# ZooMEISTER/vickers-hardness-Unet

Measured on AMD Instinct MI355X. Metric: 512x512 images/sec (train fwd+bwd), higher is better.
Workload: dtype bf16

## Files before the change

### vickers-hardness-unet_amd/csrc/conv_halo.hip

```cpp
#include <stdlib.h>
#include <string.h>

#include <string>
#include <type_traits>

#include "vk_common.h"

#ifdef VK_STAMP
#define VK_T(var) { __builtin_amdgcn_sched_barrier(0); const unsigned long long t_ = __builtin_amdgcn_s_memtime(); __builtin_amdgcn_s_waitcnt(0xC07F); __builtin_amdgcn_sched_barrier(0); var = t_; }
#else
#define VK_T(var)
#endif

namespace vk {

struct HaloSrc {
  const void* ptr;
  const float* scale;
  const float* shift;
  int C, up, relu;
  uint32_t bytes;
};

#ifndef VK_EPI_BATCH_READS
// ... 1294 lines not shown
  const uint32_t slab_bytes = (uint32_t)p.K * 64u;
  const uint32_t lane16 = (uint32_t)lane * 16u;
  auto dma_b = [&](int cc, int s, int buf) {
#pragma unroll
    for (int i = 0; i < Cfg::DMAW; ++i) {
      const int pc = wave + i * NW;
      const int r = pc / (BN / 16), sub = pc - r * (BN / 16);
      const int tap = p.flip ? 8 - (3 * r + s) : 3 * r + s;
      const uint32_t goff = (uint32_t)(cc * 9 + tap) * slab_bytes + (uint32_t)(n0 + sub * 16) * 64u;
      char* dst = Bbuf + buf * Cfg::B_BYTES + (r * BN + sub * 16) * 64;
      __builtin_amdgcn_raw_ptr_buffer_load_lds(rsw, (lds_void*)dst, 16, lane16, goff, 0, 0);
    }
  };

  const int wrow0 = (wave / WGN) * TP;
  const int wch0 = (wave % WGN) * (TC * 16);
  f32x4_t acc[TC][TP];
#pragma unroll
  for (int a = 0; a < TC; ++a)
#pragma unroll
    for (int b = 0; b < TP; ++b) acc[a][b] = f32x4_t{0.f, 0.f, 0.f, 0.f};
  const int li = lane & 15, kg = lane >> 4;
  const int a_lane = (wrow0 * 18 + li) * APS + kg * 16;
  const int b_lane = (wch0 + li) * 64 + ((kg ^ swz(li)) << 4);

  u32x4_t X[TP + 2], W0[TC], W1[TC], W2[TC];
  auto rd = [](const char* q) { return *reinterpret_cast<const u32x4_t*>(q); };
  auto mfma_row = [&](const u32x4_t (&Wr)[TC], int r) {
#pragma unroll
    for (int a = 0; a < TC; ++a)
#pragma unroll
      for (int b = 0; b < TP; ++b) acc[a][b] = Mma<T>::run(Wr[a], X[b + r], acc[a][b]);
  };
  constexpr int NM = TC * TP * (sizeof(T) == 4 ? 4 : 1);
  constexpr int kWaitAll = 0x0070;
  constexpr int kWaitLds = 0xC07F;

#ifdef VK_STAMP
  unsigned long long t_begin, t_pro, tkX = 0, tkW = 0, tkB1 = 0, tkY = 0, tkB2 = 0;
  VK_T(t_begin)
#endif
  const int ksp = p.ksplit > 1 ? p.ksplit : 1;
  const int c_begin = (int)((long)p.nchunks * blockIdx.z / ksp), c_end = (int)((long)p.nchunks * (blockIdx.z + 1) / ksp);
  load_halo(c_begin);
  dma_b(c_begin, 0, 0);
  dma_b(c_begin, 1, 1);
  dma_b(c_begin, 2, 2);
  store_halo(Abuf);
  __syncthreads();
#pragma unroll
  for (int h = 0; h < TP; ++h) X[h] = rd(Abuf + a_lane + h * (18 * APS));
#pragma unroll
  for (int a = 0; a < TC; ++a) W0[a] = rd(Bbuf + b_lane + (a * 16) * 64);

  VK_T(t_pro)
  const bool late = wave >= NW / 2;
  if (late) {
    asm volatile("" ::: "memory");
    __builtin_amdgcn_s_waitcnt(kWaitLds);
    __builtin_amdgcn_s_barrier();
    asm volatile("" ::: "memory");
  }
  for (int cc = c_begin; cc < c_end; ++cc) {
    const bool next_chunk = cc + 1 < c_end;
    const char* const Acur = Abuf + ((cc - c_begin) & 1) * Cfg::A_BYTES + a_lane;
    char* const Anext = Abuf + ((cc - c_begin + 1) & 1) * Cfg::A_BYTES;
#pragma unroll
    for (int s = 0; s < 3; ++s) {
      const int st = 3 * (cc - c_begin) + s;
      const char* const As = Acur + s * APS;
      const char* const Bs = Bbuf + (st & 3) * Cfg::B_BYTES + b_lane;
      const bool more = s < 2 || next_chunk;
      const char* const An = s < 2 ? Acur + (s + 1) * APS : Anext + a_lane;
      const char* const Bn = Bbuf + ((st + 1) & 3) * Cfg::B_BYTES + b_lane;
#ifdef VK_STAMP
      unsigned long long t0, t1, t2, t3, t4, t5;
#endif
      VK_T(t0)
      X[TP] = rd(As + TP * (18 * APS));
#pragma unroll
      for (int a = 0; a < TC; ++a) W1[a] = rd(Bs + (BN + a * 16) * 64);
      X[TP + 1] = rd(As + (TP + 1) * (18 * APS));
#pragma unroll
      for (int a = 0; a < TC; ++a) W2[a] = rd(Bs + (2 * BN + a * 16) * 64);
      mfma_row(W0, 0);
      mfma_row(W1, 1);
      mfma_row(W2, 2);
      __builtin_amdgcn_sched_group_barrier(0x100, 2 + 2 * TC, 0);
      __builtin_amdgcn_sched_group_barrier(0x008, 3 * NM, 0);
      VK_T(t1)
      asm volatile("" ::: "memory");
      __builtin_amdgcn_s_waitcnt(kWaitAll);
      VK_T(t2)
      __builtin_amdgcn_s_barrier();
      asm volatile("" ::: "memory");
      VK_T(t3)
      if (p.dbg & 16) __builtin_amdgcn_s_setprio(1);
      if (more) {
#pragma unroll
        for (int h = 0; h < TP; ++h) X[h] = rd(An + h * (18 * APS));
#pragma unroll
        for (int a = 0; a < TC; ++a) W0[a] = rd(Bn + (a * 16) * 64);
      }
      __builtin_amdgcn_sched_barrier(0);
      if (next_chunk) {
        if (s == 0) load_halo(cc + 1);
        if (s == 1) store_halo(Anext);
        dma_b(cc + 1, s, (st + 3) & 3);
      }
      asm volatile("" ::: "memory");
      __builtin_amdgcn_s_waitcnt(kWaitLds);
      if (p.dbg & 16) __builtin_amdgcn_s_setprio(0);
      VK_T(t4)
      __builtin_amdgcn_s_barrier();
      asm volatile("" ::: "memory");
      VK_T(t5)
#ifdef VK_STAMP
      tkX += t1 - t0; tkW += t2 - t1; tkB1 += t3 - t2; tkY += t4 - t3; tkB2 += t5 - t4;
#endif
    }
  }
  if (!late) {
    asm volatile("" ::: "memory");
    __builtin_amdgcn_s_barrier();
    asm volatile("" ::: "memory");
  }
  __builtin_amdgcn_s_waitcnt(kWaitAll);
#ifdef VK_STAMP
  {
    unsigned long long t_end;
    VK_T(t_end)
    if (p.stamps && lane == 0) {
      unsigned long long* o = p.stamps + ((size_t)(blockIdx.y * gridDim.x + blockIdx.x) * NW + wave) * 8;
      o[0] = tkX; o[1] = tkW; o[2] = tkB1; o[3] = tkY; o[4] = tkB2; o[5] = t_pro - t_begin; o[6] = t_end - t_begin; o[7] = 3 * (c_end - c_begin);
    }
  }
#endif
  __syncthreads();

  if (p.ksplit > 1) {
    float* sl = p.slab + (size_t)blockIdx.z * ((size_t)p.N * p.H * p.W * p.K);
#pragma unroll
    for (int a = 0; a < TC; ++a)
#pragma unroll
      for (int b = 0; b < TP; ++b) {
        const int y = y0 + wrow0 + b, x = x0 + li, ch = n0 + wch0 + a * 16 + kg * 4;
        if (y < p.H && x < p.W && ch < p.K) *reinterpret_cast<f32x4_t*>(sl + (((size_t)n * p.H + y) * p.W + x) * p.K + ch) = acc[a][b];
      }
    return;
  }
  halo_epilogue<T, TH, BN, TP, TC, NT, (BN <= 64 && TH == 16)>(smem, acc, p, n, y0, x0, n0, wrow0, wch0);
}

template <typename T, int TH, int BN, int WGM, int WGN, int MINW>
__global__ __launch_bounds__(64 * WGM * WGN, MINW) void conv3x3_colp_kernel(const HaloParams p) {
  using Cfg = ColCfg<T, TH, BN, WGM, WGN, false>;
  constexpr int EB = Cfg::EB, VE = Cfg::VE, CK = Cfg::CK, HPIX = Cfg::HPIX, NPV = Cfg::NPV, NT = Cfg::NT, NW = Cfg::NW;
  constexpr int TP = Cfg::TP, TC = Cfg::TC, APS = Cfg::APS, NPIECE = Cfg::NPIECE;
  typedef __attribute__((address_space(3))) void lds_void;

  extern __shared__ __attribute__((aligned(16))) char smem[];
  char* const Abuf = smem;
  char* const Bbuf = smem + Cfg::A_BYTES;
  const int tid = threadIdx.x, lane = tid & 63;
  const int wave = __builtin_amdgcn_readfirstlane(tid >> 6);
  const int nsp = p.N * p.tiles_y * p.tiles_x;
  const int total = nsp * p.kyn;
  const bool xcd_runs = (nsp & 7) == 0 && (gridDim.x & 7) == 0 && p.kyn == 1;

  const __amdgpu_buffer_rsrc_t rs0 = make_rsrc(p.s0.ptr, p.s0.bytes);
  const __amdgpu_buffer_rsrc_t rs1 = make_rsrc(p.s1.ptr ? p.s1.ptr : p.s0.ptr, p.s1.ptr ? p.s1.bytes : 0u);
  const __amdgpu_buffer_rsrc_t rsw = make_rsrc(p.w, p.w_bytes);

  const int hv = tid & 3;
  const int hgrp = halo_group(tid);
  const int Hh = p.H >> 1, Wh = p.W >> 1;
  struct TileGeo { int n, y0, x0, n0; };
  auto decode = [&](int t) {
    TileGeo g;
    const int ky = t % p.kyn;
    int bt = t / p.kyn;
    if (xcd_runs) bt = (bt & 7) * (nsp >> 3) + (bt >> 3);
    const int tx = bt % p.tiles_x;
    bt /= p.tiles_x;
    const int ty = bt % p.tiles_y;
    g.n = bt / p.tiles_y;
    g.y0 = ty * TH; g.x0 = tx * 16; g.n0 = ky * BN;
    return g;
  };
  auto halo_index = [&](const TileGeo& g, int (&hf)[NPV], int (&hh)[NPV]) {
#pragma unroll
    for (int i = 0; i < NPV; ++i) {
      const int hp = hgrp + i * (NT / 4);
      const int hy = hp / 18, hx = hp - hy * 18;
      const int y = g.y0 - 1 + hy, x = g.x0 - 1 + hx;
      const bool ok = hp < HPIX && (unsigned)y < (unsigned)p.H && (unsigned)x < (unsigned)p.W;
      hf[i] = ok ? (g.n * p.H + y) * p.W + x : -1;
      hh[i] = ok ? (g.n * Hh + (y >> 1)) * Wh + (x >> 1) : -1;
    }
  };
  int h_full[NPV], h_half[NPV], h_full_n[NPV], h_half_n[NPV];
  u32x4_t areg[NPV];
  float sc[VE], sh[VE];
  bool aff = false, relu = false;

  auto load_halo = [&](int cc, const int (&hf)[NPV], const int (&hh)[NPV]) {
    const int c = cc * CK;
    const bool first = c < p.s0.C;
    const HaloSrc& sd = first ? p.s0 : p.s1;
    const int cl = (first ? c : c - p.s0.C) + hv * VE;
    aff = sd.scale != nullptr;
    relu = sd.relu != 0;
    if (aff) {
#pragma unroll
      for (int j = 0; j < VE; j += 4) {
        const f32x4_t s4 = *reinterpret_cast<const f32x4_t*>(sd.scale + cl + j);
        const f32x4_t h4 = *reinterpret_cast<const f32x4_t*>(sd.shift + cl + j);
#pragma unroll
        for (int e = 0; e < 4; ++e) { sc[j + e] = s4[e]; sh[j + e] = h4[e]; }
      }
    }
    const bool up = sd.up != 0;
#pragma unroll
    for (int i = 0; i < NPV; ++i) {
      const int pix = up ? hh[i] : hf[i];
      const uint32_t off = (uint32_t)(pix * sd.C + cl) * (uint32_t)EB;
      if (first) areg[i] = buf_load16(rs0, pix >= 0 ? off : kOOB);
      else areg[i] = buf_load16(rs1, pix >= 0 ? off : kOOB);
    }
  };
  auto store_halo = [&](char* A, const int (&hf)[NPV]) {
#pragma unroll
    for (int i = 0; i < NPV; ++i) {
      const int hp = hgrp + i * (NT / 4);
      if (hp >= HPIX) continue;
      u32x4_t v = areg[i];
      if (aff) {
        v = AffineRelu<T>::run(v, sc, sh, relu);
        if (hf[i] < 0) v = u32x4_t{0, 0, 0, 0};
      }
      *reinterpret_cast<u32x4_t*>(A + hp * APS + hv * 16) = v;
    }
  };
  const uint32_t slab_bytes = (uint32_t)p.K * 64u;
  const uint32_t lane16 = (uint32_t)lane * 16u;
  auto dma_b = [&](int n0, int cc, int s, int buf) {
#pragma unroll
    for (int i = 0; i < (NPIECE + NW - 1) / NW; ++i) {
      const int pc = wave + i * NW;
      if (NPIECE % NW == 0 || pc < NPIECE) {
        const int r = pc / (BN / 16), sub = pc - r * (BN / 16);
        const int tap = p.flip ? 8 - (3 * r + s) : 3 * r + s;
        const uint32_t goff = (uint32_t)(cc * 9 + tap) * slab_bytes + (uint32_t)(n0 + sub * 16) * 64u;
        char* dst = Bbuf + buf * Cfg::B_BYTES + (r * BN + sub * 16) * 64;
        __builtin_amdgcn_raw_ptr_buffer_load_lds(rsw, (lds_void*)dst, 16, lane16, goff, 0, 0);
      }
    }
  };

  const int wrow0 = (wave / WGN) * TP;
  const int wch0 = (wave % WGN) * (TC * 16);
  const int li = lane & 15, kg = lane >> 4;
  const int a_lane = (wrow0 * 18 + li) * APS + kg * 16;
  const int b_lane = (wch0 + li) * 64 + ((kg ^ swz(li)) << 4);
  f32x4_t acc[TC][TP];

  auto compute = [&](const char* A, const char* B) {
    u32x4_t X[TP + 2], W[3][TC];
#pragma unroll
    for (int h = 0; h < TP + 2; ++h) X[h] = *reinterpret_cast<const u32x4_t*>(A + h * (18 * APS));
#pragma unroll
    for (int r = 0; r < 3; ++r)
#pragma unroll
      for (int a = 0; a < TC; ++a) W[r][a] = *reinterpret_cast<const u32x4_t*>(B + (r * BN + a * 16) * 64);
#pragma unroll
    for (int r = 0; r < 3; ++r)
#pragma unroll
      for (int a = 0; a < TC; ++a)
#pragma unroll
        for (int b = 0; b < TP; ++b) acc[a][b] = Mma<T>::run(W[r][a], X[b + r], acc[a][b]);
    constexpr int NM = TC * TP * (sizeof(T) == 4 ? 4 : 1);
    __builtin_amdgcn_sched_group_barrier(0x100, TP + 2 + TC, 0);
    __builtin_amdgcn_sched_group_barrier(0x100, TC, 0);
    __builtin_amdgcn_sched_group_barrier(0x008, NM, 0);
    __builtin_amdgcn_sched_group_barrier(0x100, TC, 0);
    __builtin_amdgcn_sched_group_barrier(0x008, NM, 0);
    __builtin_amdgcn_sched_group_barrier(0x008, NM, 0);
  };

  int t = blockIdx.x;
  if (t >= total) return;
  TileGeo g = decode(t);
  halo_index(g, h_full, h_half);
  load_halo(0, h_full, h_half);
  double dsum[2] = {0.0, 0.0};
  int st = 0;
  for (;;) {
    dma_b(g.n0, 0, 0, st & 1);
    store_halo(Abuf, h_full);
    __syncthreads();
#pragma unroll
    for (int a = 0; a < TC; ++a)
#pragma unroll
      for (int b = 0; b < TP; ++b) acc[a][b] = f32x4_t{0.f, 0.f, 0.f, 0.f};
    const int tn = t + (int)gridDim.x;
    const bool more_tiles = tn < total;
    TileGeo gn = g;
    const char* const A = Abuf + a_lane;
    auto stage = [&](int cc, auto s_c, auto last_c) {
      constexpr int s = decltype(s_c)::value;
      constexpr bool LAST = decltype(last_c)::value;
      if (s < 2) dma_b(g.n0, cc, s + 1, (st + 1) & 1);
      else if (!LAST) dma_b(g.n0, cc + 1, 0, (st + 1) & 1);
      if (s == 0 && !LAST) load_halo(cc + 1, h_full, h_half);
      if (s == 2 && LAST && more_tiles) {
        gn = decode(tn);
        halo_index(gn, h_full_n, h_half_n);
        load_halo(0, h_full_n, h_half_n);
      }
      compute(A + s * APS, Bbuf + (st & 1) * Cfg::B_BYTES + b_lane);
      if (s == 2 && !LAST) {
        __syncthreads();
        store_halo(Abuf, h_full);
      }
      __syncthreads();
      ++st;
    };
    using I0 = std::integral_constant<int, 0>;
    using I1 = std::integral_constant<int, 1>;
    using I2 = std::integral_constant<int, 2>;
    for (int cc = 0; cc + 1 < p.nchunks; ++cc) {
      stage(cc, I0{}, std::false_type{});
      stage(cc, I1{}, std::false_type{});
      stage(cc, I2{}, std::false_type{});
    }
    stage(p.nchunks - 1, I0{}, std::true_type{});
    stage(p.nchunks - 1, I1{}, std::true_type{});
    stage(p.nchunks - 1, I2{}, std::true_type{});
    constexpr bool DEFER = VK_COLP_DEFER_STATS && (sizeof(T) == 2 || BN < 64);
    halo_epilogue<T, TH, BN, TP, TC, NT, (BN <= 64 && TH == 16)>(smem, acc, p, g.n, g.y0, g.x0, g.n0, wrow0, wch0, 0, 0, DEFER ? dsum : nullptr);
    if (DEFER && (!more_tiles || gn.n0 != g.n0)) stats_flush<BN>(p, g.n0, dsum);
    if (!more_tiles) break;
    __syncthreads();
    t = tn;
    g = gn;
#pragma unroll
    for (int i = 0; i < NPV; ++i) { h_full[i] = h_full_n[i]; h_half[i] = h_half_n[i]; }
  }
}

struct StemTile {
  static constexpr int ROWS = 37, VPR = 20, PITCH = VPR * 16;
  static constexpr int A_BYTES = ROWS * PITCH;
  static constexpr int W_OFF = (A_BYTES + 1023) / 1024 * 1024, W_BYTES = 28 * 1024;
};

template <typename T>
__global__ __launch_bounds__(256, 3) void stem7x7_kernel(const HaloParams p) {
  using Cfg = ColCfg<T, 16, 64, 4, 1, false>;
  static_assert(sizeof(T) == 2, "16-bit types: a pixel of the NHWC4 input is 8 bytes");
  constexpr int NV = (StemTile::ROWS * StemTile::VPR + 255) / 256;
  extern __shared__ __attribute__((aligned(16))) char smem[];
  const int tid = threadIdx.x, lane = tid & 63;
  const int wave = __builtin_amdgcn_readfirstlane(tid >> 6);
  int bt = blockIdx.x;
  if ((gridDim.x & 7) == 0) bt = (bt & 7) * (int)(gridDim.x >> 3) + (bt >> 3);
  const int tx = bt % p.tiles_x;
  bt /= p.tiles_x;
  const int ty = bt % p.tiles_y;
  const int n = bt / p.tiles_y;
  const int y0 = ty * 16, x0 = tx * 16;
  const __amdgpu_buffer_rsrc_t rs0 = make_rsrc(p.s0.ptr, p.s0.bytes);
  const __amdgpu_buffer_rsrc_t rsw = make_rsrc(p.w, p.w_bytes);

  u32x4_t areg[NV];
#pragma unroll
  for (int i = 0; i < NV; ++i) {
    const int v = tid + i * 256;
    const int ry = v / StemTile::VPR, vc = v - ry * StemTile::VPR;
    const int y = 2 * y0 - 3 + ry, x = 2 * x0 - 4 + 2 * vc;
    const bool ok = v < StemTile::ROWS * StemTile::VPR && (unsigned)y < (unsigned)p.Hi && (unsigned)x < (unsigned)p.Wi;
    areg[i] = buf_load16(rs0, ok ? (uint32_t)((n * p.Hi + y) * p.Wi + x) * 8u : kOOB);
  }
  const int li = lane & 15, kg = lane >> 4;
  typedef __attribute__((address_space(3))) void lds_void;
  char* const Wl = smem + StemTile::W_OFF;
#pragma unroll
  for (int i = 0; i < 7; ++i) {
    const int pc = wave * 7 + i, r = pc >> 2, a = pc & 3;
    const uint32_t voff = (uint32_t)((((a * 16 + li) * 7 + r) * 32 + kg * 8) * 2);
    __builtin_amdgcn_raw_ptr_buffer_load_lds(rsw, (lds_void*)(Wl + pc * 1024), 16, voff, 0, 0, 0);
  }
#pragma unroll
  for (int i = 0; i < NV; ++i) {
    const int v = tid + i * 256;
    if (v >= StemTile::ROWS * StemTile::VPR) continue;
    const int ry = v / StemTile::VPR, vc = v - ry * StemTile::VPR;
    char* row = smem + ry * StemTile::PITCH;
    if (vc > 0) *reinterpret_cast<u32x2_t*>(row + (2 * vc - 1) * 8) = u32x2_t{areg[i][0], areg[i][1]};
    *reinterpret_cast<u32x2_t*>(row + (2 * vc) * 8) = u32x2_t{areg[i][2], areg[i][3]};
  }
  __syncthreads();

  const int wrow0 = wave * 4;
  f32x4_t acc[4][4];
#pragma unroll
  for (int a = 0; a < 4; ++a)
#pragma unroll
    for (int b = 0; b < 4; ++b) acc[a][b] = f32x4_t{0.f, 0.f, 0.f, 0.f};
  const char* const xl = smem + (2 * wrow0) * StemTile::PITCH + 16 * (li + kg);
  const char* const wl = Wl + lane * 16;
#pragma unroll
  for (int r = 0; r < 7; ++r) {
    u32x4_t X[4], Wc[4];
#pragma unroll
    for (int a = 0; a < 4; ++a) Wc[a] = *reinterpret_cast<const u32x4_t*>(wl + (4 * r + a) * 1024);
#pragma unroll
    for (int b = 0; b < 4; ++b) X[b] = *reinterpret_cast<const u32x4_t*>(xl + (2 * b + r) * StemTile::PITCH);
#pragma unroll
    for (int a = 0; a < 4; ++a)
#pragma unroll
      for (int b = 0; b < 4; ++b) acc[a][b] = Mma<T>::run(Wc[a], X[b], acc[a][b]);
  }
  __syncthreads();
  halo_epilogue<T, 16, 64, 4, 4, 256, false>(smem, acc, p, n, y0, x0, 0, wrow0, 0);
}

int stem_tile_launch(vk_dtype dt, int N, int H, int W, const void* x4, const void* wp, void* y, double* stats, hipStream_t st) {
  if (dt == VK_F32 || getenv("VK_NO_STEM_TILE")) return VK_ERR_UNSUPPORTED;
  if ((size_t)N * H * W * 8 >= (1ull << 31)) return VK_ERR_UNSUPPORTED;
  HaloParams p;
  memset((void*)&p, 0, sizeof(p));
  p.s0 = HaloSrc{x4, nullptr, nullptr, 4, 0, 0, (uint32_t)((size_t)N * H * W * 8)};
  p.w = wp;
  p.w_bytes = 64u * 7u * 32u * 2u;
  p.y0 = y;
  p.ld0 = 64;
  p.stats = stats;
  p.N = N; p.H = H / 2; p.W = W / 2; p.K = 64; p.C = 4;
  p.Hi = H; p.Wi = W;
  p.tiles_x = (p.W + 15) / 16;
  p.tiles_y = (p.H + 15) / 16;
  using Cfg = ColCfg<bf16_t, 16, 64, 4, 1, false>;
  constexpr int MAIN = StemTile::W_OFF + StemTile::W_BYTES;
  constexpr int SMEM = MAIN > Cfg::EPI ? MAIN : Cfg::EPI;
  const dim3 grid((unsigned)(N * p.tiles_y * p.tiles_x));
  vkh::ProfScope ps("stem_tile_16b", st, 2.0 * (double)N * p.H * p.W * 64.0 * 147.0, ((double)N * H * W * 4.0 + (double)N * p.H * p.W * 64.0) * 2.0);
  if (dt == VK_BF16) hipLaunchKernelGGL(stem7x7_kernel<bf16_t>, grid, dim3(256), SMEM, st, p);
  else hipLaunchKernelGGL(stem7x7_kernel<f16_t>, grid, dim3(256), SMEM, st, p);
  VK_CHECK_HIP(hipGetLastError());
  return VK_OK;
}

template <typename T, int BN>
struct C16Cfg {
  static constexpr int TH = 16, HPIX = 18 * 18;
  static constexpr int APS = 48;
  static constexpr int A_BYTES = HPIX * APS + 64;
  static constexpr int BS = 336;
  static constexpr int B_BYTES = BN * BS;
  static constexpr int TP = 4, TC = BN / 16;
  static constexpr int ESB = BN * 2 + 16;
  static constexpr int EPI = 256 * ESB + 4 * 4 * BN * 2 * 4;
  static constexpr int MAIN = A_BYTES + B_BYTES;
  static constexpr int SMEM = MAIN > EPI ? MAIN : EPI;
};

template <typename T, int BN>
__global__ __launch_bounds__(256) void conv3x3_c16_kernel(const HaloParams p) {
  using Cfg = C16Cfg<T, BN>;
  constexpr int TH = 16, HPIX = Cfg::HPIX, APS = Cfg::APS, BS = Cfg::BS, TP = Cfg::TP, TC = Cfg::TC, VE = 8;
  static_assert(sizeof(T) == 2, "C16 kernel is for 16-bit element types (fp32 uses the generic kernel with 16-channel chunks)");
  extern __shared__ __attribute__((aligned(16))) char smem[];
  char* const Abuf = smem;
  char* const Bbuf = smem + Cfg::A_BYTES;
  const int tid = threadIdx.x, lane = tid & 63, wave = tid >> 6;
  int bt = blockIdx.x;
// ... 580 lines not shown
  vkh::ProfScope ps("dec4_tail_eval_16b", st, 2.0 * px * (9.0 * 32 * 16 + 9.0 * 16 * 16 + 144.0), px * (32.0 * 2 / 4 + 4.0));
  if (dt == VK_BF16) hipLaunchKernelGGL(dec4_tail_eval_kernel<bf16_t>, dim3(nb), dim3(256), TailCfg::SMEM, st, p);
  else hipLaunchKernelGGL(dec4_tail_eval_kernel<f16_t>, dim3(nb), dim3(256), TailCfg::SMEM, st, p);
  VK_CHECK_HIP(hipGetLastError());
  return VK_OK;
}

template <typename T>
__global__ void k_pack_halo(int rows, int red, const T* __restrict__ src, T* __restrict__ dst) {
  constexpr int CK = 64 / ElemTraits<T>::kBytes, VE = ElemTraits<T>::kVec;
  const size_t total = (size_t)rows * 9 * red / VE;
  for (size_t v = blockIdx.x * (size_t)blockDim.x + threadIdx.x; v < total; v += (size_t)gridDim.x * blockDim.x) {
    const int pos = (int)(v & 3);
    size_t t = v >> 2;
    const int k = (int)(t % rows);
    t /= rows;
    const int tap = (int)(t % 9);
    const int cc = (int)(t / 9);
    const int j = pos ^ (((k >> 2) & 1) << 1);
    const u32x4_t x = *reinterpret_cast<const u32x4_t*>(src + ((size_t)k * 9 + tap) * red + cc * CK + j * VE);
    *reinterpret_cast<u32x4_t*>(dst + v * VE) = x;
  }
}

int halo_pack_impl(vk_dtype dt, int rows, int red, const void* src, void* dst, hipStream_t st) {
  const int eb = dt == VK_F32 ? 4 : 2;
  VK_CHECK_ARG(src && dst && rows > 0 && red % (64 / eb) == 0, "vk_halo_pack: reduction channels %d must be a multiple of %d", red, 64 / eb);
  const size_t nvec = (size_t)rows * 9 * red * eb / 16;
  unsigned nb = (unsigned)((nvec + 255) / 256);
  if (nb > 4096) nb = 4096;
  switch (dt) {
    case VK_F32: hipLaunchKernelGGL(k_pack_halo<float>, dim3(nb), dim3(256), 0, st, rows, red, (const float*)src, (float*)dst); break;
    case VK_BF16: hipLaunchKernelGGL(k_pack_halo<bf16_t>, dim3(nb), dim3(256), 0, st, rows, red, (const bf16_t*)src, (bf16_t*)dst); break;
    case VK_F16: hipLaunchKernelGGL(k_pack_halo<f16_t>, dim3(nb), dim3(256), 0, st, rows, red, (const f16_t*)src, (f16_t*)dst); break;
  }
  VK_CHECK_HIP(hipGetLastError());
  return VK_OK;
}

template <typename T, int TH, int BN, int WGM, int WGN>
static int launch_halo(HaloParams p, hipStream_t st) {
  using Cfg = HaloCfg<T, TH, BN, WGM, WGN>;
  p.tiles_x = (p.W + 15) / 16;
  p.tiles_y = (p.H + TH - 1) / TH;
  dim3 grid((unsigned)(p.N * p.tiles_y * p.tiles_x), (unsigned)((p.K + BN - 1) / BN), 1);
  static bool attr_done = false;
  if (!attr_done && Cfg::SMEM > 64 * 1024) {
    VK_CHECK_HIP(hipFuncSetAttribute((const void*)conv3x3_halo_kernel<T, TH, BN, WGM, WGN>,
                                     hipFuncAttributeMaxDynamicSharedMemorySize, Cfg::SMEM));
    attr_done = true;
  }
  {
    static const std::string tag_f = std::string("halo_") + (sizeof(T) == 4 ? "f32" : "16b") + "_t" + std::to_string(TH) + "_bn" + std::to_string(BN);
    static const std::string tag_d = tag_f + "_dgrad";
    const double macs = (double)p.N * p.H * p.W * p.K * 9.0 * p.C;
    const double bytes = ((double)p.N * p.H * p.W * (p.C + p.K) + 9.0 * p.K * p.C) * sizeof(T);
    const std::string& btag = p.flip ? tag_d : tag_f;
    const std::string dtag = getenv("VK_PROF_DETAIL") ? btag + ":H" + std::to_string(p.H) + "_K" + std::to_string(p.K) + "_C" + std::to_string(p.C) : btag;
    vkh::ProfScope ps(dtag.c_str(), st, 2.0 * macs, bytes);
    hipLaunchKernelGGL((conv3x3_halo_kernel<T, TH, BN, WGM, WGN>), grid, dim3(256), Cfg::SMEM, st, p);
  }
  VK_CHECK_HIP(hipGetLastError());
  return VK_OK;
}

template <typename T>
__global__ __launch_bounds__(256) void k_splitk_reduce(size_t n4, int splits, const float* __restrict__ slab, T* __restrict__ y) {
  const size_t e = blockIdx.x * (size_t)blockDim.x + threadIdx.x;
  if (e >= n4) return;
  f32x4_t a = *reinterpret_cast<const f32x4_t*>(slab + e * 4);
  for (int s = 1; s < splits; ++s) a = a + *reinterpret_cast<const f32x4_t*>(slab + ((size_t)s * n4 + e) * 4);
  if constexpr (sizeof(T) == 4) {
    *reinterpret_cast<f32x4_t*>(y + e * 4) = a;
  } else {
    float f[8] = {a[0], a[1], a[2], a[3], 0.f, 0.f, 0.f, 0.f};
    const u32x4_t pk = Vec16<T>::pack(f);
    *reinterpret_cast<u32x2_t*>(y + e * 4) = u32x2_t{pk[0], pk[1]};
  }
}

template <int PIPE, typename T, int TH, int BN, int WGM, int WGN, bool ADB, int MINW, int STR>
struct ColLaunch {
  using Cfg = ColCfg<T, TH, BN, WGM, WGN, ADB, STR>;
  static const void* kernel() { return (const void*)conv3x3_col_kernel<T, TH, BN, WGM, WGN, ADB, MINW, STR>; }
};
template <typename T, int TH, int BN, int WGM, int WGN, bool ADB, int MINW>
struct ColLaunch<1, T, TH, BN, WGM, WGN, ADB, MINW, 1> {
  using Cfg = ColqCfg<T, TH, BN, WGM, WGN>;
  static const void* kernel() { return (const void*)conv3x3_colq_kernel<T, TH, BN, WGM, WGN>; }
};
template <typename T, int TH, int BN, int WGM, int WGN, bool ADB, int MINW>
struct ColLaunch<2, T, TH, BN, WGM, WGN, ADB, MINW, 1> {
  using Cfg = ColsCfg<T, TH, BN, WGM, WGN>;
  static const void* kernel() { return (const void*)conv3x3_cols_kernel<T, TH, BN, WGM, WGN>; }
};

template <typename T, int TH, int BN, int WGM, int WGN, bool ADB, int MINW, int PIPE = 0, int STR = 1>
static int launch_col(HaloParams p, hipStream_t st) {
  using Sel = ColLaunch<PIPE, T, TH, BN, WGM, WGN, ADB, MINW, STR>;
  using Cfg = typename Sel::Cfg;
  const void* const kernel = Sel::kernel();
  p.tiles_x = (p.W + 15) / 16;
  p.tiles_y = (p.H + TH - 1) / TH;
  dim3 grid((unsigned)(p.N * p.tiles_y * p.tiles_x), (unsigned)((p.K + BN - 1) / BN), 1);
  const size_t out_elems = (size_t)p.N * p.H * p.W * p.K;
  int ks = 1;
  if (p.slab && !p.stats && !p.bnr_z && !p.accumulate && !p.pool2 && p.split == 0 && !getenv("VK_NO_SPLITK")) {
    const long wgs = (long)grid.x * grid.y;
    const char* force = getenv("VK_SPLITK");
    ks = force ? atoi(force) : (wgs < 128 ? (int)(256 / wgs) : 1);
    if (ks > p.nchunks / 2) ks = p.nchunks / 2;
    if (ks > 32) ks = 32;
    while (ks > 1 && (size_t)ks * out_elems * sizeof(float) > p.slab_bytes) --ks;
    if (ks < 2) ks = 1;
  }
  p.ksplit = ks;
  grid.z = (unsigned)ks;
  p.kyn = 0;
  if (ks == 1 && grid.y > 1 && (grid.x & 7) == 0 && !getenv("VK_COL_NO_KYFAST")) {
    p.kyn = (int)grid.y;
    grid.x *= grid.y;
    grid.y = 1;
    const char* km = getenv("VK_COL_KYMODE");
    const bool wst = km ? km[0] == 'w' : (size_t)p.w_bytes >= (3u << 20);
    if (PIPE && wst && 8 % p.kyn == 0 && (grid.x / 8) * (8 / p.kyn) * p.kyn == grid.x) p.kyn = -p.kyn;
  }
  static bool attr_done = false;
  if (!attr_done && Cfg::SMEM > 64 * 1024) {
    VK_CHECK_HIP(hipFuncSetAttribute(kernel, hipFuncAttributeMaxDynamicSharedMemorySize, Cfg::SMEM));
    attr_done = true;
  }
  {
    static const std::string tag_f = std::string(PIPE == 2 ? "cols_" : PIPE == 1 ? "colq_" : "col_") + (sizeof(T) == 4 ? "f32" : "16b") + "_t" + std::to_string(TH) + "_bn" +
                                     std::to_string(BN) + "_w" + std::to_string(WGM * WGN) + (STR == 2 ? "_s2" : "");
    static const std::string tag_d = tag_f + "_dgrad";
    const double macs = (double)p.N * p.H * p.W * p.K * 9.0 * p.C;
    const double bytes = ((double)p.N * ((double)p.Hi * p.Wi * p.C + (double)p.H * p.W * p.K) + 9.0 * p.K * p.C) * sizeof(T);
    const std::string& btag = p.flip ? tag_d : tag_f;
    const std::string dtag = getenv("VK_PROF_DETAIL") ? btag + ":H" + std::to_string(p.H) + "_K" + std::to_string(p.K) + "_C" + std::to_string(p.C) : btag;
    vkh::ProfScope ps(dtag.c_str(), st, 2.0 * macs, bytes);
    void* args[] = {(void*)&p};
    VK_CHECK_HIP(hipLaunchKernel(kernel, grid, dim3(Cfg::NT), args, Cfg::SMEM, st));
  }
  if (ks > 1) {
    vkh::ProfScope ps("splitk_reduce", st, 0.0, (double)out_elems * (4.0 * ks + sizeof(T)));
    hipLaunchKernelGGL(k_splitk_reduce<T>, dim3((unsigned)((out_elems / 4 + 255) / 256)), dim3(256), 0, st, out_elems / 4, ks, p.slab, (T*)p.y0);
  }
  VK_CHECK_HIP(hipGetLastError());
  return VK_OK;
}

template <typename T, int TH, int BN, int WGM, int WGN, int MINW>
static int launch_colp(HaloParams p, hipStream_t st) {
  using Cfg = ColCfg<T, TH, BN, WGM, WGN, false>;
  p.tiles_x = (p.W + 15) / 16;
  p.tiles_y = (p.H + TH - 1) / TH;
  p.kyn = (p.K + BN - 1) / BN;
  p.ksplit = 1;
  const long total = (long)p.N * p.tiles_y * p.tiles_x * p.kyn;
  int per_cu = (160 * 1024) / Cfg::SMEM;
  if (per_cu > 4) per_cu = 4;
  if (per_cu < 1) per_cu = 1;
  long g = 256L * per_cu;
  if (const char* e = getenv("VK_COL_PERSIST_GRID")) g = atol(e) > 0 ? atol(e) : g;
  if (g > total) g = total;
  static bool attr_done = false;
  if (!attr_done && Cfg::SMEM > 64 * 1024) {
    VK_CHECK_HIP(hipFuncSetAttribute((const void*)conv3x3_colp_kernel<T, TH, BN, WGM, WGN, MINW>,
                                     hipFuncAttributeMaxDynamicSharedMemorySize, Cfg::SMEM));
    attr_done = true;
  }
  {
    static const std::string tag_f = std::string("col_") + (sizeof(T) == 4 ? "f32" : "16b") + "_t" + std::to_string(TH) + "_bn" + std::to_string(BN) +
                                     "_w" + std::to_string(WGM * WGN);
    static const std::string tag_d = tag_f + "_dgrad";
    const double macs = (double)p.N * p.H * p.W * p.K * 9.0 * p.C;
    const double bytes = ((double)p.N * p.H * p.W * (p.C + p.K) + 9.0 * p.K * p.C) * sizeof(T);
    const std::string& btag = p.flip ? tag_d : tag_f;
    const std::string dtag = getenv("VK_PROF_DETAIL") ? btag + ":H" + std::to_string(p.H) + "_K" + std::to_string(p.K) + "_C" + std::to_string(p.C) : btag;
    vkh::ProfScope ps(dtag.c_str(), st, 2.0 * macs, bytes);
    hipLaunchKernelGGL((conv3x3_colp_kernel<T, TH, BN, WGM, WGN, MINW>), dim3((unsigned)g), dim3(Cfg::NT), Cfg::SMEM, st, p);
  }
  VK_CHECK_HIP(hipGetLastError());
  return VK_OK;
}

template <typename T, int BN>
static int launch_small(const HaloParams& p, hipStream_t st) {
  const long total = (long)p.N * ((p.H + 15) / 16) * ((p.W + 15) / 16) * ((p.K + BN - 1) / BN);
  const char* pe = getenv("VK_COL_PERSIST");
  const long min_tiles = pe ? (atol(pe) == 0 ? -1 : atol(pe)) : (BN == 64 ? 1024 : -1);
  const bool splitk_wanted = p.slab && !p.stats && !p.bnr_z && !p.accumulate && !p.pool2 && p.split == 0 && total < 128;
  if (min_tiles > 0 && !splitk_wanted && total >= min_tiles) return launch_colp<T, 16, BN, 4, 1, 2>(p, st);
  return launch_col<T, 16, BN, 4, 1, false, 2>(p, st);
}

template <typename T>
static int col_select(const HaloParams& p, hipStream_t st) {
  const char* alt_s = getenv("VK_COL_ALT");
  const int alt = alt_s ? atoi(alt_s) : 0;
  const long tiles16 = (long)p.N * ((p.H + 15) / 16) * ((p.W + 15) / 16);
  if (p.K >= 128) {
    const long kt = (p.K + 127) / 128;
    if (alt == 1) return launch_col<T, 16, 128, 2, 2, true, 1>(p, st);
    if (alt == 8 || (alt == 0 && p.nchunks <= 2 && p.K % 128 != 0) || (alt == 0 && p.nchunks == 1)) return launch_small<T, 64>(p, st);
    if (alt == 3 || (alt != 2 && alt != 7 && p.nchunks <= 2)) return launch_col<T, 8, 128, 2, 2, false, 2>(p, st);
    const char* const pipe_s = getenv("VK_COL_PIPE");
    const int pipe = pipe_s ? atoi(pipe_s) : 1;
    if (alt == 7 || (alt != 2 && tiles16 * kt < 256))
      return pipe == 2 ? launch_col<T, 8, 128, 2, 4, true, 1, 2>(p, st)
             : pipe    ? launch_col<T, 8, 128, 2, 4, true, 1, 1>(p, st) : launch_col<T, 8, 128, 2, 4, true, 2>(p, st);
    if (alt == 9) return launch_col<T, 16, 128, 2, 4, true, 1, 1>(p, st);
    return pipe == 2 ? launch_col<T, 16, 128, 4, 2, true, 1, 2>(p, st)
           : pipe    ? launch_col<T, 16, 128, 4, 2, true, 1, 1>(p, st) : launch_col<T, 16, 128, 4, 2, true, 2>(p, st);
  }
  if (p.K >= 64) return launch_small<T, 64>(p, st);
  if (p.K >= 32) return launch_small<T, 32>(p, st);
  return launch_small<T, 16>(p, st);
}

template <typename T>
static int halo_select(const HaloParams& p, hipStream_t st) {
  const bool old_loop = getenv("VK_HALO_ROWSTAGED") != nullptr;
  if (!old_loop) return col_select<T>(p, st);
  const long tiles8 = (long)p.N * ((p.H + 7) / 8) * ((p.W + 15) / 16);
  const long tiles16 = (long)p.N * ((p.H + 15) / 16) * ((p.W + 15) / 16);
  if (p.K >= 128) {
    if (tiles8 * ((p.K + 127) / 128) >= 512) return launch_halo<T, 8, 128, 2, 2>(p, st);
    return launch_halo<T, 8, 64, 2, 2>(p, st);
  }
  if (p.K >= 64) {
    if (tiles16 >= 1024) return launch_halo<T, 16, 64, 4, 1>(p, st);
    return launch_halo<T, 8, 64, 2, 2>(p, st);
  }
  if (p.K >= 32) return launch_halo<T, 16, 32, 4, 1>(p, st);
  return launch_halo<T, 16, 16, 4, 1>(p, st);
}

template <typename T, int BN>
static int launch_c16(HaloParams p, hipStream_t st) {
  using Cfg = C16Cfg<T, BN>;
  p.tiles_x = (p.W + 15) / 16;
  p.tiles_y = (p.H + 15) / 16;
  dim3 grid((unsigned)(p.N * p.tiles_y * p.tiles_x), (unsigned)((p.K + BN - 1) / BN), 1);
  {
    static const std::string tag_f = std::string("c16_16b_bn") + std::to_string(BN);
    static const std::string tag_d = tag_f + "_dgrad";
    const std::string& btag = p.flip ? tag_d : tag_f;
    const double bytes = ((double)p.N * p.H * p.W * (16.0 + p.K * (p.pool2 ? 0.25 : 1.0)) + 9.0 * p.K * 16.0) * 2.0;
    vkh::ProfScope ps(btag.c_str(), st, 2.0 * (double)p.N * p.H * p.W * p.K * 144.0, bytes);
    hipLaunchKernelGGL((conv3x3_c16_kernel<T, BN>), grid, dim3(256), Cfg::SMEM, st, p);
  }
  VK_CHECK_HIP(hipGetLastError());
  return VK_OK;
}

template <typename T, int BN>
static int launch_s2dg(HaloParams p, hipStream_t st) {
  using Cfg = S2dCfg<T, 8, BN, 4, 2>;
  p.tiles_x = (p.Wi + 15) / 16;
  p.tiles_y = (p.Hi + 7) / 8;
  dim3 grid((unsigned)(p.N * p.tiles_y * p.tiles_x), (unsigned)((p.K + BN - 1) / BN), 1);
  static bool attr_done = false;
  if (!attr_done && Cfg::SMEM > 64 * 1024) {
    VK_CHECK_HIP(hipFuncSetAttribute((const void*)conv3x3_s2dg_kernel<T, 8, BN, 4, 2>, hipFuncAttributeMaxDynamicSharedMemorySize, Cfg::SMEM));
    attr_done = true;
  }
  {
    static const std::string tag = std::string("s2dg_") + (sizeof(T) == 4 ? "f32" : "16b") + "_bn" + std::to_string(BN);
    const std::string dtag = getenv("VK_PROF_DETAIL") ? tag + ":H" + std::to_string(p.H) + "_K" + std::to_string(p.K) + "_C" + std::to_string(p.C) : tag;
    const double bytes = ((double)p.N * ((double)p.Hi * p.Wi * p.C + (double)p.H * p.W * p.K * (p.accumulate ? 2.0 : 1.0)) + 9.0 * p.K * p.C) * sizeof(T);
    vkh::ProfScope ps(dtag.c_str(), st, 2.0 * (double)p.N * p.Hi * p.Wi * p.K * 9.0 * p.C, bytes);
    hipLaunchKernelGGL((conv3x3_s2dg_kernel<T, 8, BN, 4, 2>), grid, dim3(Cfg::NT), Cfg::SMEM, st, p);
  }
  VK_CHECK_HIP(hipGetLastError());
  return VK_OK;
}

template <typename T, int CIN, int TC, bool UP, int MODE>
static int launch_stream(const HaloParams& p, hipStream_t st) {
  using Cfg = StreamCfg<T, CIN, UP>;
  HaloParams q = p;
  const char* e_rs = getenv("VK_STREAM_RS");
  int RS = Cfg::RS;
  if (e_rs) {
    RS = atoi(e_rs);
  } else {
    const long per_row_block = (long)p.N * ((p.W + 15) / 16);
    while (RS * 2 <= 256 && per_row_block * ((p.H + 2 * RS - 1) / (2 * RS)) >= 4096) RS *= 2;
  }
  RS = (RS + 7) & ~7;
  if (RS < 8) RS = 8;
  q.tiles_y = RS;
  const long strips = (long)p.N * ((p.H + RS - 1) / RS) * ((p.W + 15) / 16);
  dim3 grid((unsigned)((strips + 3) / 4), 1, 1);
  static const std::string tag_f = std::string("stream_16b_c") + std::to_string(CIN) + (UP ? "up" : "") + "_k" + std::to_string(TC * 16);
  static const std::string tag_d = tag_f + "_dgrad";
  const std::string& tag = p.flip ? tag_d : tag_f;
  const double in_px = (double)p.N * (p.H >> (UP ? 1 : 0)) * (p.W >> (UP ? 1 : 0));
  const double out_px = (double)p.N * p.H * p.W * (p.pool2 ? 0.25 : 1.0);
  const double bytes = (in_px * CIN + out_px * p.K * (p.bnr_z ? 2.0 : 1.0) + 9.0 * p.K * CIN) * 2.0;
  vkh::ProfScope ps(tag.c_str(), st, 2.0 * (double)p.N * p.H * p.W * p.K * 9.0 * CIN, bytes);
  hipLaunchKernelGGL((conv3x3_stream_kernel<T, CIN, TC, UP, MODE>), grid, dim3(256), Cfg::SMEM, st, q);
  VK_CHECK_HIP(hipGetLastError());
  return VK_OK;
}

// ... 121 lines not shown
```

Before: 2993.

## Double-buffer halo tile in colp conv kernel with XOR-swizzled LDS layout

Gives the persistent 3x3 conv kernel two A (halo) buffers in LDS instead of one, so the next channel chunk's halo is stored during stage 1 into the alternate buffer. This removes the extra barrier before storing the halo at the end of each chunk. The halo rows drop their padded pitch and use a dense 64-byte pitch with an XOR swizzle to avoid LDS bank conflicts. It costs more LDS, and a static assert checks that two workgroups still fit per CU.

After: 2991, median of 6. Within noise of the previous version (-0.1%).

```diff
diff --git a/vickers-hardness-unet_amd/csrc/conv_halo.hip b/vickers-hardness-unet_amd/csrc/conv_halo.hip
--- a/vickers-hardness-unet_amd/csrc/conv_halo.hip
+++ b/vickers-hardness-unet_amd/csrc/conv_halo.hip
@@ -1470,16 +1470,26 @@
   halo_epilogue<T, TH, BN, TP, TC, NT, (BN <= 64 && TH == 16)>(smem, acc, p, n, y0, x0, n0, wrow0, wch0);
 }
 
+template <typename T, int TH, int BN, int WGM, int WGN>
+struct ColpCfg : ColCfg<T, TH, BN, WGM, WGN, false> {
+  using Base = ColCfg<T, TH, BN, WGM, WGN, false>;
+  static constexpr int RP = 18 * 64;
+  static constexpr int A_BYTES = Base::HH * RP;
+  static constexpr int MAIN = 2 * A_BYTES + 2 * Base::B_BYTES;
+  static constexpr int SMEM = MAIN > Base::EPI ? MAIN : Base::EPI;
+  static_assert(Base::HWI == 18 && 2 * SMEM <= 160 * 1024, "two workgroups per CU");
+};
+
 template <typename T, int TH, int BN, int WGM, int WGN, int MINW>
 __global__ __launch_bounds__(64 * WGM * WGN, MINW) void conv3x3_colp_kernel(const HaloParams p) {
-  using Cfg = ColCfg<T, TH, BN, WGM, WGN, false>;
+  using Cfg = ColpCfg<T, TH, BN, WGM, WGN>;
   constexpr int EB = Cfg::EB, VE = Cfg::VE, CK = Cfg::CK, HPIX = Cfg::HPIX, NPV = Cfg::NPV, NT = Cfg::NT, NW = Cfg::NW;
-  constexpr int TP = Cfg::TP, TC = Cfg::TC, APS = Cfg::APS, NPIECE = Cfg::NPIECE;
+  constexpr int TP = Cfg::TP, TC = Cfg::TC, RP = Cfg::RP, NPIECE = Cfg::NPIECE;
   typedef __attribute__((address_space(3))) void lds_void;
 
   extern __shared__ __attribute__((aligned(16))) char smem[];
   char* const Abuf = smem;
-  char* const Bbuf = smem + Cfg::A_BYTES;
+  char* const Bbuf = smem + 2 * Cfg::A_BYTES;
   const int tid = threadIdx.x, lane = tid & 63;
   const int wave = __builtin_amdgcn_readfirstlane(tid >> 6);
   const int nsp = p.N * p.tiles_y * p.tiles_x;
@@ -1491,7 +1501,12 @@
   const __amdgpu_buffer_rsrc_t rsw = make_rsrc(p.w, p.w_bytes);
 
   const int hv = tid & 3;
-  const int hgrp = halo_group(tid);
+  const int hgrp = tid >> 2;
+  int swzm = 0;
+#pragma unroll
+  for (int i = 0; i < NPV; ++i) swzm |= (swz((hgrp + i * (NT / 4)) % 18) >> 1) << i;
+#pragma unroll
+  for (int s = 0; s < 3; ++s) swzm |= (swz((tid & 15) + s) >> 1) << (8 + s);
   const int Hh = p.H >> 1, Wh = p.W >> 1;
   struct TileGeo { int n, y0, x0, n0; };
   auto decode = [&](int t) {
@@ -1548,6 +1563,8 @@
     }
   };
   auto store_halo = [&](char* A, const int (&hf)[NPV]) {
+    int m = swzm;
+    asm volatile("" : "+v"(m));
 #pragma unroll
     for (int i = 0; i < NPV; ++i) {
       const int hp = hgrp + i * (NT / 4);
@@ -1557,7 +1574,7 @@
         v = AffineRelu<T>::run(v, sc, sh, relu);
         if (hf[i] < 0) v = u32x4_t{0, 0, 0, 0};
       }
-      *reinterpret_cast<u32x4_t*>(A + hp * APS + hv * 16) = v;
+      *reinterpret_cast<u32x4_t*>(A + i * (NT / 4) * 64 + ((hgrp * 64 + hv * 16) ^ (((m >> i) & 1) << 5))) = v;
     }
   };
   const uint32_t slab_bytes = (uint32_t)p.K * 64u;
@@ -1579,14 +1596,14 @@
   const int wrow0 = (wave / WGN) * TP;
   const int wch0 = (wave % WGN) * (TC * 16);
   const int li = lane & 15, kg = lane >> 4;
-  const int a_lane = (wrow0 * 18 + li) * APS + kg * 16;
+  const int a_lane = (wrow0 * 18 + li) * 64 + kg * 16;
   const int b_lane = (wch0 + li) * 64 + ((kg ^ swz(li)) << 4);
   f32x4_t acc[TC][TP];
 
   auto compute = [&](const char* A, const char* B) {
     u32x4_t X[TP + 2], W[3][TC];
 #pragma unroll
-    for (int h = 0; h < TP + 2; ++h) X[h] = *reinterpret_cast<const u32x4_t*>(A + h * (18 * APS));
+    for (int h = 0; h < TP + 2; ++h) X[h] = *reinterpret_cast<const u32x4_t*>(A + h * RP);
 #pragma unroll
     for (int r = 0; r < 3; ++r)
 #pragma unroll
@@ -1624,7 +1641,6 @@
     const int tn = t + (int)gridDim.x;
     const bool more_tiles = tn < total;
     TileGeo gn = g;
-    const char* const A = Abuf + a_lane;
     auto stage = [&](int cc, auto s_c, auto last_c) {
       constexpr int s = decltype(s_c)::value;
       constexpr bool LAST = decltype(last_c)::value;
@@ -1636,11 +1652,11 @@
         halo_index(gn, h_full_n, h_half_n);
         load_halo(0, h_full_n, h_half_n);
       }
-      compute(A + s * APS, Bbuf + (st & 1) * Cfg::B_BYTES + b_lane);
-      if (s == 2 && !LAST) {
-        __syncthreads();
-        store_halo(Abuf, h_full);
-      }
+      int m = swzm;
+      asm volatile("" : "+v"(m));
+      compute(Abuf + (cc & 1) * Cfg::A_BYTES + s * 64 + (a_lane ^ (((m >> (8 + s)) & 1) << 5)),
+              Bbuf + (st & 1) * Cfg::B_BYTES + b_lane);
+      if (s == 1 && !LAST) store_halo(Abuf + ((cc + 1) & 1) * Cfg::A_BYTES, h_full);
       __syncthreads();
       ++st;
     };
@@ -2527,7 +2543,7 @@
 
 template <typename T, int TH, int BN, int WGM, int WGN, int MINW>
 static int launch_colp(HaloParams p, hipStream_t st) {
-  using Cfg = ColCfg<T, TH, BN, WGM, WGN, false>;
+  using Cfg = ColpCfg<T, TH, BN, WGM, WGN>;
   p.tiles_x = (p.W + 15) / 16;
   p.tiles_y = (p.H + TH - 1) / TH;
   p.kyn = (p.K + BN - 1) / BN;
```
